# yangzhaojason/DualDiff

Hardware: AMD Instinct MI355X
Metric: denoising-steps/sec, 6-view 224×400 fp16, 50-step DDIM @ 1/2/4/8 MI355X (higher is better)
Workload: dtype fp16; 1 GPU; BASELINE configs[1]: 6-view 224x400 (28x50 latents) multiview UNet + 2 ControlNet branches (ORS panorama + ORS-3D, SFA on), CFG 2.0 -> 12 view-instances/scene, DDIM-50 schedule, random-init weights; scenes_per_gpu=1, parallelism=scene-sharded x1 (no data-path collective), hip_graph=True, streams=3, invariant_conditioning=recomputed every step

## Files before the change

### dualdiff_amd/_native.py

```python
import ctypes
import os

import torch
from ctypes import (POINTER, Structure, c_char_p, c_float, c_int32, c_int64, c_uint32, c_void_p)

from . import _build

DD_F16, DD_BF16, DD_F32 = 0, 1, 2
DD_EPI_NONE, DD_EPI_GEGLU, DD_EPI_SILU = 0, 1, 2


class GemmDesc(Structure):
    _fields_ = [
        ("a", c_void_p), ("a2", c_void_p), ("lda", c_int64), ("lda2", c_int64), ("k1", c_int32),
        ("rows", c_int32), ("n", c_int32), ("k", c_int32),
        ("w", c_void_p), ("bias", c_void_p), ("rowvec", c_void_p),
        ("rows_per_inst", c_int32), ("ld_rowvec", c_int32),
        ("res", c_void_p), ("ldres", c_int64),
        ("out", c_void_p), ("ldc", c_int64),
        ("alpha", c_float), ("accumulate", c_int32), ("epilogue", c_int32),
        ("conv", c_int32), ("hin", c_int32), ("win", c_int32), ("cin", c_int32),
        ("hv", c_int32), ("wv", c_int32), ("hout", c_int32), ("wout", c_int32), ("stride", c_int32),
        ("dtype", c_int32), ("tile", c_int32), ("split_k", c_int32),
        ("ws", c_void_p), ("ws_bytes", c_int64),
        ("ln_colsum", c_void_p), ("ln_bias", c_void_p), ("ln_eps", c_float), ("out_f32", c_int32), ("ln_stats_out", c_void_p), ("ln_stats_in", c_void_p),
        ("out_headmajor_d", c_int32), ("hm_scaled_planes", c_int32), ("hm_scale", c_float),
        ("phase", c_int32),
        ("ln_out", c_void_p), ("ld_ln_out", c_int64), ("lno_gamma", c_void_p), ("lno_beta", c_void_p),
    ]


class AttnDesc(Structure):
    _fields_ = [
        ("q", c_void_p), ("k", c_void_p), ("v", c_void_p), ("o", c_void_p),
        ("ldq", c_int64), ("ldk", c_int64), ("ldv", c_int64), ("ldo", c_int64),
        ("q_batch_stride", c_int64), ("k_batch_stride", c_int64),
        ("v_batch_stride", c_int64), ("o_batch_stride", c_int64),
        ("batch", c_int32), ("heads", c_int32), ("head_dim", c_int32), ("lq", c_int32), ("lk", c_int32),
        ("scale", c_float),
        ("kv_batch_map", c_void_p),
        ("accumulate", c_int32), ("dtype", c_int32), ("variant", c_int32),
        ("q_head_stride", c_int64), ("k_head_stride", c_int64), ("v_head_stride", c_int64),
        ("q_prescaled", c_int32),
# ... 35 lines not shown
        ("w", c_void_p), ("w_scale", c_void_p), ("ldw", c_int64),
        ("bias", c_void_p), ("res", c_void_p), ("ldres", c_int64),
        ("out", c_void_p), ("ldc", c_int64),
        ("rows", c_int32), ("n", c_int32), ("k_padded", c_int32), ("dtype", c_int32),
        ("out_headmajor_d", c_int32), ("hm_scaled_planes", c_int32), ("hm_scale", c_float), ("geglu", c_int32),
    ]


SIGNATURES = {
    "dd_abi_version": (c_int32, []),
    "dd_desc_size": (c_int64, [c_int32]),
    "dd_error_string": (c_char_p, [c_int32]),
    "dd_target_arch": (c_char_p, []),
    "dd_gemm": (c_int32, [POINTER(GemmDesc), c_void_p]),
    "dd_gemm_workspace_bytes": (c_int64, [POINTER(GemmDesc)]),
    "dd_gemm_num_tiles": (c_int32, []),
    "dd_gemm_tile_id": (c_int32, [c_int32]),
    "dd_gemm_kernel_name": (c_char_p, [POINTER(GemmDesc)]),
    "dd_groupnorm_nhwc": (c_int32, [c_void_p, c_int32, c_void_p, c_int32, c_void_p, c_void_p, c_void_p,
                                    c_int32, c_int32, c_int32, c_float, c_int32, c_int32,
                                    c_void_p, c_int64, c_void_p]),
    "dd_groupnorm_workspace_bytes": (c_int64, [c_int32, c_int32]),
    "dd_groupnorm_is_fused": (c_int32, [c_int32, c_int32, c_int32]),
    "dd_layernorm": (c_int32, [c_void_p, c_void_p, c_void_p, c_void_p, c_int64, c_int32, c_float,
                               c_int32, c_void_p]),
    "dd_attention": (c_int32, [POINTER(AttnDesc), c_void_p]),
    "dd_attention_kernel_name": (c_char_p, [POINTER(AttnDesc)]),
    "dd_add": (c_int32, [c_void_p, c_void_p, c_void_p, c_void_p, c_int64, c_int32, c_void_p]),
    "dd_scale": (c_int32, [c_void_p, c_void_p, c_float, c_int64, c_int32, c_void_p]),
    "dd_probe_spin": (c_int32, [c_void_p, c_uint32, c_void_p]),
    "dd_groupnorm_splitk": (c_int32, [c_void_p, c_int32, c_void_p, c_void_p, c_int32, c_void_p, c_int64, c_void_p,
                                      c_void_p, c_void_p, c_void_p, c_int32, c_int32, c_int32, c_int32, c_float, c_int32,
                                      c_int32, c_void_p]),
    "dd_xattn320": (c_int32, [POINTER(XAttnDesc), c_void_p]),
    "dd_nchw_to_nhwc_views": (c_int32, [c_void_p, c_void_p, c_int32, c_int32, c_int32, c_int32, c_int32, c_int32, c_int32,
                                        c_void_p]),
    "dd_fourier_embed_strided": (c_int32, [c_void_p, c_void_p, c_int64, c_int32, POINTER(c_float), c_int32, c_int32,
                                           c_int32, c_int32, c_int32, c_int64, c_int64, c_int64, c_int64, c_void_p]),
# ... 82 lines not shown
```

### dualdiff_amd/csrc/dd_common.h

```cpp
#pragma once
#include <hip/hip_runtime.h>
#include <stdint.h>
#include <atomic>
#include "../../include/dualdiff_hip.h"

typedef float f32x4 __attribute__((ext_vector_type(4)));
typedef _Float16 f16x8 __attribute__((ext_vector_type(8)));
typedef __bf16 bf16x8 __attribute__((ext_vector_type(8)));
typedef _Float16 f16x4 __attribute__((ext_vector_type(4)));
typedef __bf16 bf16x4 __attribute__((ext_vector_type(4)));
typedef short s16x4 __attribute__((ext_vector_type(4)));
typedef uint32_t u32x4 __attribute__((ext_vector_type(4)));
typedef uint32_t u32x2 __attribute__((ext_vector_type(2)));

#define DD_WAVE 64

template <typename T> struct dd_vec;
template <> struct dd_vec<_Float16> { using v8 = f16x8; using v4 = f16x4; };
template <> struct dd_vec<__bf16>   { using v8 = bf16x8; using v4 = bf16x4; };

__device__ __forceinline__ f32x4 dd_mfma16(f16x8 a, f16x8 b, f32x4 c) {
#ifdef DD_DBG_NOMFMA
  asm volatile("" ::"v"(a), "v"(b));
  return c;
// ... 59 lines not shown
__device__ __forceinline__ float dd_geglu_f(float h, float g) {
#ifdef DD_DBG_GEGLU_CHEAP
  return h * g;
#endif
  const float ax = fabsf(g);
  const float t = __builtin_amdgcn_rcpf(fmaf(0.3275911f * 0.70710678118654752440f, ax, 1.0f));
  float p = fmaf(0.5f * 1.061405429f, t, 0.5f * -1.453152027f);
  p = fmaf(p, t, 0.5f * 1.421413741f);
  p = fmaf(p, t, 0.5f * -0.284496736f);
  p = fmaf(p, t, 0.5f * 0.254829592f);
  const float e = __builtin_amdgcn_exp2f((-0.5f * 1.4426950408889634f) * (g * g));
  const float q = (p * t) * e;
  return h * fmaf(-ax, q, fmaxf(g, 0.0f));
}

__device__ __forceinline__ float dd_wave_sum(float v) {
#pragma unroll
  for (int o = 32; o > 0; o >>= 1) v += __shfl_xor(v, o, 64);
  return v;
}
__device__ __forceinline__ float dd_wave_max(float v) {
#pragma unroll
  for (int o = 32; o > 0; o >>= 1) v = fmaxf(v, __shfl_xor(v, o, 64));
  return v;
}

static inline void dd_clear_error() { (void)hipGetLastError(); }
static inline int dd_check_launch() {
  return hipGetLastError() == hipSuccess ? DD_OK : DD_ERR_LAUNCH;
}
// ... 12 lines not shown
```

### dualdiff_amd/csrc/gemm.hip

```cpp
#include "dd_common.h"
#include "dd_debug.h"
#include <type_traits>

namespace {

constexpr int BK = 64;

struct GemmParams {
  const void* a; const void* a2; int64_t lda, lda2; int k1;
  int rows, n, k;
  const void* w; const void* bias; const void* rowvec; int rows_per_inst, ld_rowvec;
  const void* res; int64_t ldres;
  void* out; int64_t ldc;
  float alpha; int accumulate; int act;
  int hin, win, cin, hv, wv, hout, wout, stride, upsample;
  float scale_h, scale_w;
  int k_per_split;
  float* partial;
  int tiles_m, tiles_n;
  uint32_t a_bytes, a2_bytes, w_bytes;
  uint32_t out_bytes, res_bytes;
  int g_per_tile, chunks_per_split;
  int band_rows, bands; float inv_bands;
  const float* ln_colsum; const float* ln_bias; float ln_eps;
  int out_f32;
  float* stat_out;
  const float* stat_in;
  int hm_d, hm_planes; float hm_scale;
  int persist;
  uint64_t* dbg_stamps;
  float inv_hw, inv_wout, inv_rpi;
  void* ln_out; int64_t ld_ln_out;
  const void* lno_gamma; const void* lno_beta;
  float inv_tiles_n, inv_hm_d;
  uint32_t ln_out_bytes;
};

__device__ __forceinline__ int dd_fdiv(int n, float inv) { return (int)(((float)n + 0.5f) * inv); }


template <typename T>
__device__ __forceinline__ void store8(const GemmParams& p, int64_t row, int col, float (&v)[8]) {
  if (p.hm_d) {
    const int plane = col / p.hm_d;
    if (plane < p.hm_planes) {
#pragma unroll
      for (int e = 0; e < 8; ++e) v[e] *= p.hm_scale;
    }
    dd_st16(reinterpret_cast<T*>(p.out) + ((int64_t)plane * p.rows + row) * p.hm_d + (col - plane * p.hm_d),
            dd_pack8<T>(v));
// ... 42 lines not shown
    for (int i = 0; i < 8; ++i) v[i] += b[i];
  }
  store8<T>(p, row, col, v);
}

__device__ __forceinline__ int xcd_remap(int bid, int nwg) {
  const int xcd = bid & 7;
  const int q = nwg >> 3, r = nwg & 7;
  const int base = (xcd < r) ? xcd * (q + 1) : r * (q + 1) + (xcd - r) * q;
  return base + (bid >> 3);
}

template <typename T, int TM, int TN, bool GEGLU>
__device__ __forceinline__ void store_tile(const GemmParams& p, f32x4 (&acc)[TN][TM], int block_m0,
                                           int block_n0, int wave_m, int wave_n, int lane, int row_end,
                                           const float* ln_mean = nullptr, const float* ln_rstd = nullptr) {
  const int q = lane >> 4;
  const int c = lane & 15;
  const int row0 = block_m0 + wave_m * (TM * 16) + c;
  if constexpr (GEGLU) {
    constexpr int TH = TN / 2;
    constexpr int NG = TH / 2;
    const int col0 = block_n0 + wave_n * (TH * 16) + q * (4 * TH);
    u32x4 bh[NG], bg[NG];
    f32x4 lsh[NG][2], lsg[NG][2], lbh[NG][2], lbg[NG][2];
    if (ln_mean) {
#pragma unroll
      for (int g8 = 0; g8 < NG; ++g8) {
        const int col = min(col0 + g8 * 8, p.n - 8);
#pragma unroll
        for (int h2 = 0; h2 < 2; ++h2) {
// ... 58 lines not shown
      for (int tm = 0; tm < TM; ++tm) {
        const int row = row0 + tm * 16;
        if (row >= row_end) continue;
#pragma unroll
        for (int g8 = 0; g8 < NG; ++g8) {
          const int col = col0 + g8 * 8;
          if (col >= p.n) continue;
          float* dst = p.partial + ((int64_t)blockIdx.z * p.rows + row) * p.n + col;
          *reinterpret_cast<f32x4*>(dst) = acc[g8 * 2][tm];
          *reinterpret_cast<f32x4*>(dst + 4) = acc[g8 * 2 + 1][tm];
        }
      }
      return;
    }
    constexpr int TMB = (TM >= 4 && TM % 2 == 0) ? TM / 2 : TM;
    u32x4 rb[NG];
    int colc[NG];
#pragma unroll
    for (int g8 = 0; g8 < NG; ++g8) colc[g8] = min(col0 + g8 * 8, p.n - 8);
    if (p.bias) {
#pragma unroll
      for (int g8 = 0; g8 < NG; ++g8) rb[g8] = dd_ld16(reinterpret_cast<const T*>(p.bias) + colc[g8]);
    }
    f32x4 lcs[NG][2], lcb[NG][2];
    if (ln_mean) {
#pragma unroll
      for (int g8 = 0; g8 < NG; ++g8)
#pragma unroll
        for (int h2 = 0; h2 < 2; ++h2) {
          lcs[g8][h2] = *reinterpret_cast<const f32x4*>(p.ln_colsum + colc[g8] + 4 * h2);
// ... 55 lines not shown
#pragma unroll
          for (int e = 0; e < 8; ++e) v[e] *= p.alpha;
          if (p.res) {
            dd_unpack8<T>(rr[t2][g8], b);
#pragma unroll
            for (int e = 0; e < 8; ++e) v[e] += b[e];
          }
          if (p.act == DD_EPI_SILU) {
#pragma unroll
            for (int e = 0; e < 8; ++e) v[e] = dd_silu_f(v[e]);
          }
          if (p.accumulate) {
            dd_unpack8<T>(ra[t2][g8], b);
#pragma unroll
            for (int e = 0; e < 8; ++e) v[e] += b[e];
          }
          store8<T>(p, row, col, v);
          if (p.stat_out) {
#pragma unroll
            for (int e = 0; e < 8; ++e) { st_s += v[e]; st_q += v[e] * v[e]; }
          }
        }
        }
        if constexpr (TN == 2 || TN == 4) {
          if (p.stat_out) {
            st_s += __shfl_xor(st_s, 16, 64);  st_q += __shfl_xor(st_q, 16, 64);
            if (TN == 2) { st_s += __shfl_xor(st_s, 32, 64);  st_q += __shfl_xor(st_q, 32, 64); }
            const int gcol = block_n0 + wave_n * (TN * 16) + (TN == 2 ? 0 : (q >> 1) * 32);
            const bool writer = TN == 2 ? q == 0 : (q & 1) == 0;
            if (writer && row < row_end && gcol < p.n) {
              float* dst = p.stat_out + ((int64_t)row * (p.n >> 5) + (gcol >> 5)) * 2;
              dst[0] = st_s;
              dst[1] = st_q;
            }
          }
        }
      }
    }
  }
}

template <typename T, int WAVES_M, int WAVES_N, int TM, int TN, bool CONV, bool GEGLU>
__global__ __launch_bounds__(64 * WAVES_M * WAVES_N)
void dd_gemm_kernel(const GemmParams p) {
  using V8 = typename dd_vec<T>::v8;
  constexpr int NT = 64 * WAVES_M * WAVES_N;
  constexpr int BM = WAVES_M * TM * 16;
  constexpr int BN = WAVES_N * TN * 16;
  constexpr int BN_OUT = GEGLU ? BN / 2 : BN;
  constexpr int XI = BM * 8 / NT;
  constexpr int WI = BN * 8 / NT;
// ... 1735 lines not shown
  if constexpr (NW == 8 && GRP == 1) {
    if (late) main_loop(std::true_type{});
    else main_loop(std::false_type{});
  } else {
    main_loop(std::false_type{});
  }
  DD_STAMP(4);
  if (late && nsteps > 0) {
#pragma unroll
    for (int j = 0; j < TM; ++j)
#pragma unroll
      for (int ks = 0; ks < 2; ++ks)
#pragma unroll
        for (int i = 0; i < TN; ++i) acc[i][j] = C3_MFMA(wf[ks][i], xf[ks][j], acc[i][j]);
  }
  store_tile<T, TM, TN, false>(p, acc, row0, block_n0, wave_m, wave_n, lane, min(p.rows, row0 + vrows));
  DD_STAMP_FLUSH(p);
  C3_SEG_FLUSH(p, wave, lane, nsteps);
}

template <typename T>
__global__ __launch_bounds__(256)
void dd_splitk_reduce_kernel(const GemmParams p, int nsplit) {
  const int64_t groups_per_row = p.n / 8;
  const int64_t total = (int64_t)p.rows * groups_per_row;
  for (int64_t g = (int64_t)blockIdx.x * blockDim.x + threadIdx.x; g < total;
       g += (int64_t)gridDim.x * blockDim.x) {
    const int row = (int)(g / groups_per_row);
    const int col = (int)(g - (int64_t)row * groups_per_row) * 8;
    float v[8] = {0, 0, 0, 0, 0, 0, 0, 0};
    for (int z = 0; z < nsplit; ++z) {
// ... 422 lines not shown

}

extern "C" int dd_gemm_num_tiles(void) { return kNumTiles; }
extern "C" int dd_gemm_tile_id(int index) { return (index >= 0 && index < kNumTiles) ? kTiles[index].id : -1; }

constexpr int64_t DD_COUNTER_BYTES = 65536;

extern "C" int64_t dd_gemm_workspace_bytes(const dd_gemm_desc* d) {
  if (validate(d) != DD_OK) return 0;
  const Plan pl = make_plan(d);
  if (pl.unsupported || pl.split <= 1) return 0;
  return DD_COUNTER_BYTES + (int64_t)pl.split * d->rows * d->n * (int64_t)sizeof(float);
}

extern "C" const char* dd_gemm_kernel_name(const dd_gemm_desc* d) {
  if (validate(d) != DD_OK) return "invalid";
  const Plan pl = make_plan(d);
  if (pl.unsupported) return "unsupported";
  const TileCfg& t = kTiles[pl.tile_idx];
  if (t.stages < 0) {
    const bool band = t.stages == -3;
    const int nsw = (t.id == 31 || band) ? 5 : (t.id >= 37 ? 6 : (t.id >= 35 ? 3 : 4));
    snprintf(g_kname, sizeof(g_kname), "dd_conv3s_kernel<%s, %d, %d, %d, %d, %d, %d, %s> split=%d grid=%dx%d tile=%s",
             d->dtype == DD_F16 ? "_Float16" : "__bf16", t.wm, t.wn, t.tm, t.tn, nsw, (t.id >= 37 && !band) ? 3 : 1,
             band ? "true" : "false", pl.split, pl.tiles_m, pl.tiles_n, t.name);
    return g_kname;
  }
  if (t.stages >= 100) {
    snprintf(g_kname, sizeof(g_kname), "dd_gemm%d_kernel<%s, %d, %d, %d, %d, %d, %s> split=%d grid=%dx%d tile=%s",
// ... 54 lines not shown
      p.a2_bytes = d->a2 ? (uint32_t)((((int64_t)d->rows - 1) * d->lda2 + (d->k - d->k1)) * 2) : 0u;
    }
  }
  {
    const int64_t ob = (((int64_t)d->rows - 1) * d->ldc + d->n) * 2, rb = (((int64_t)d->rows - 1) * d->ldres + d->n) * 2;
    const bool fits = ob < ((int64_t)1 << 31) && (!d->res || rb < ((int64_t)1 << 31));
    p.out_bytes = fits ? (uint32_t)ob : 0u;
    p.res_bytes = fits && d->res ? (uint32_t)rb : 0u;
  }
  p.persist = 0;
  p.inv_tiles_n = 1.0f / (float)(pl.tiles_n > 0 ? pl.tiles_n : 1);
  p.inv_hm_d = d->out_headmajor_d > 0 ? 1.0f / (float)d->out_headmajor_d : 1.0f;
  p.ln_out_bytes = d->ln_out ? (uint32_t)((((int64_t)d->rows - 1) * d->ld_ln_out + d->n) * 2) : 0u;
  p.partial = nullptr;
  p.dbg_stamps = nullptr;
  DD_STAMP_HOST(p, d);
  if (pl.split > 1) {
    const int64_t need = DD_COUNTER_BYTES + (int64_t)pl.split * d->rows * d->n * (int64_t)sizeof(float);
    if (!d->ws || d->ws_bytes < need) return DD_ERR_WORKSPACE;
    p.partial = reinterpret_cast<float*>(reinterpret_cast<char*>(d->ws) + DD_COUNTER_BYTES);
  }
  hipStream_t s = reinterpret_cast<hipStream_t>(stream);
  dd_clear_error();
  if (d->dtype == DD_F16) return launch_dtype<_Float16>(d, p, pl, s);
  return launch_dtype<__bf16>(d, p, pl, s);
}
```

### dualdiff_amd/csrc/norm.hip

```cpp
#include "dd_common.h"
#include <atomic>

namespace {

constexpr int GN_THREADS = 256;
constexpr int GN_MAX_SPLIT = 64;
constexpr int GN_MAX_C = 4096;

struct GnParams {
  const void* x1; const void* x2; int c1, c2, c;
  const void* gamma; const void* beta; void* y;
  int m, hw, groups, cpg; float eps; int silu;
  float* ws;
  int nsplit, pix_per_split;
  const float* sk_part; int sk_nsplit; int64_t sk_rows;
  const void* sk_bias; const void* sk_rowvec; int sk_ld_rowvec;
  const void* sk_res; int64_t sk_ldres;
  void* sk_xout;
};

struct GnMap { int cv_count, pl_count, cv, pl; bool active; };
__device__ __forceinline__ GnMap gn_map(int c) {
  GnMap mp;
  mp.cv_count = c >> 3;
  if (mp.cv_count >= GN_THREADS) {
    mp.pl_count = 1; mp.cv = threadIdx.x; mp.pl = 0; mp.active = true;
  } else {
    mp.pl_count = GN_THREADS / mp.cv_count;
    mp.cv = threadIdx.x % mp.cv_count;
    mp.pl = threadIdx.x / mp.cv_count;
    mp.active = mp.pl < mp.pl_count;
  }
  return mp;
}
// ... 105 lines not shown
          const int t = mp.cv_count >= GN_THREADS ? (c - cv0) : pl * mp.cv_count + c;
          if (s_g0[t] == g) { gsum += s_a0[t]; gsq += s_b0[t]; }
          if (s_g1[t] == g) { gsum += s_a1[t]; gsq += s_b1[t]; }
        }
      }
    }
    __syncthreads();
  }
  if (threadIdx.x < p.groups) {
    float* dst = p.ws + (((int64_t)inst * p.nsplit + split) * p.groups + threadIdx.x) * 2;
    dst[0] = gsum;
    dst[1] = gsq;
  }
}

template <typename T>
__global__ __launch_bounds__(GN_THREADS)
void dd_gn_apply_kernel(const GnParams p) {
  __shared__ float s_mean[64], s_rstd[64];
  __shared__ float s_ps[GN_THREADS], s_pq[GN_THREADS];
  const int split = blockIdx.x, inst = blockIdx.y;
  const GnMap mp = gn_map(p.c);
  const int p0 = split * p.pix_per_split;
  const int p1 = min(p.hw, p0 + p.pix_per_split);
  const float my_pivot = (int)threadIdx.x < p.groups ? gn_pivot<T>(p, inst, threadIdx.x) : 0.f;
  const int cv_first = mp.cv;
  const int ch_first = min(cv_first, mp.cv_count - 1) << 3;
  u32x4 pre[GN_UNROLL];
  const bool pre_ok = mp.active && cv_first < mp.cv_count && p0 + mp.pl + (GN_UNROLL - 1) * mp.pl_count < p1;
  if (pre_ok) {
#pragma unroll
    for (int u = 0; u < GN_UNROLL; ++u)
      pre[u] = dd_ld16(gn_src<T>(p, (int64_t)inst * p.hw + p0 + mp.pl + u * mp.pl_count, ch_first));
  }
  {
    const int g = threadIdx.x % p.groups;
    const int chunk = threadIdx.x / p.groups;
    const int nchunk = GN_THREADS / p.groups;
    float s = 0.f, ss = 0.f;
    if (chunk < nchunk) {
      const float* src = p.ws + ((int64_t)inst * p.nsplit * p.groups + g) * 2;
      for (int i = chunk; i < p.nsplit; i += nchunk) {
        s += src[(int64_t)i * p.groups * 2];
        ss += src[(int64_t)i * p.groups * 2 + 1];
      }
    }
    s_ps[threadIdx.x] = s;
    s_pq[threadIdx.x] = ss;
    __syncthreads();
    if (threadIdx.x < p.groups) {
// ... 349 lines not shown
  int cpb, vpp, plc, nv, kred, threads;
  if (gn_fused_plan(hw, c, groups, &cpb, &vpp, &plc, &nv, &kred, &threads)) {
    dim3 fgrid(c / cpb, m);
    if (threads == 256) {
      if (dtype == DD_F16) hipLaunchKernelGGL((dd_gn_fused_kernel<_Float16, 256, GNF_NV_SMALL>), fgrid, dim3(256), 0, s, p, cpb, vpp, plc, nv, kred);
      else hipLaunchKernelGGL((dd_gn_fused_kernel<__bf16, 256, GNF_NV_SMALL>), fgrid, dim3(256), 0, s, p, cpb, vpp, plc, nv, kred);
    } else {
      if (dtype == DD_F16) hipLaunchKernelGGL((dd_gn_fused_kernel<_Float16, 1024, GNF_NV_BIG>), fgrid, dim3(1024), 0, s, p, cpb, vpp, plc, nv, kred);
      else hipLaunchKernelGGL((dd_gn_fused_kernel<__bf16, 1024, GNF_NV_BIG>), fgrid, dim3(1024), 0, s, p, cpb, vpp, plc, nv, kred);
    }
    return dd_check_launch();
  }
  dim3 grid(p.nsplit, m);
  if (dtype == DD_F16) {
    hipLaunchKernelGGL(dd_gn_stats_kernel<_Float16>, grid, dim3(GN_THREADS), 0, s, p);
    hipLaunchKernelGGL(dd_gn_apply_kernel<_Float16>, grid, dim3(GN_THREADS), 0, s, p);
  } else {
    hipLaunchKernelGGL(dd_gn_stats_kernel<__bf16>, grid, dim3(GN_THREADS), 0, s, p);
    hipLaunchKernelGGL(dd_gn_apply_kernel<__bf16>, grid, dim3(GN_THREADS), 0, s, p);
  }
  return dd_check_launch();
}

extern "C" int dd_groupnorm_splitk(const float* partial, int32_t nsplit, const void* bias, const void* rowvec,
                                   int32_t ld_rowvec, const void* res, int64_t ldres, void* x_out,
                                   const void* gamma, const void* beta, void* y, int32_t m, int32_t hw, int32_t c,
                                   int32_t groups, float eps, int32_t apply_silu, int32_t dtype, dd_stream_t stream) {
  if (!partial || !gamma || !beta || !y || nsplit < 2 || nsplit > 64) return DD_ERR_BAD_ARG;
  if (m <= 0 || hw <= 0 || groups <= 0 || groups > 64 || c <= 0 || (c & 7) || c % groups || c > GN_MAX_C) return DD_ERR_BAD_ARG;
  if (c / groups < 4) return DD_ERR_UNSUPPORTED;
  if (dtype != DD_F16 && dtype != DD_BF16) return DD_ERR_BAD_ARG;
  if (!dd_aligned16(partial) || !dd_aligned16(y) || !dd_aligned16(gamma) || !dd_aligned16(beta) ||
      (bias && !dd_aligned16(bias)) || (rowvec && (!dd_aligned16(rowvec) || (ld_rowvec & 7))) ||
      (res && (!dd_aligned16(res) || (ldres & 7))) || (x_out && !dd_aligned16(x_out))) return DD_ERR_BAD_ARG;
  int cpb, vpp, plc, nv, kred, threads;
// ... 51 lines not shown
```

### dualdiff_amd/networks/layers.py

```python
import math

import torch
import torch.nn as nn

from .. import ops as O


CACHE_EPOCH = [0]


class _Cached(nn.Module):

    def _drop_cache(self):
        CACHE_EPOCH[0] += 1
        for k in [k for k in self.__dict__ if k.startswith("_pk_")]:
            del self.__dict__[k]

    def _apply(self, fn, *a, **k):
        self._drop_cache()
        return super()._apply(fn, *a, **k)

    def _load_from_state_dict(self, *a, **k):
        self._drop_cache()
        return super()._load_from_state_dict(*a, **k)
# ... 148 lines not shown
    @property
    def cin_pad(self):
        return (self.in_channels + 7) // 8 * 8

    @property
    def packed(self):
        if "_pk_w" not in self.__dict__:
            w = self.weight.detach().permute(0, 2, 3, 1)
            if self.cin_pad != self.in_channels:
                wp = w.new_zeros((self.out_channels, 3, 3, self.cin_pad))
                wp[..., :self.in_channels] = w
                w = wp
            self.__dict__["_pk_w"] = w.reshape(self.out_channels, 9 * self.cin_pad).contiguous()
        return self.__dict__["_pk_w"]

    def run(self, x2d, m, h, w, up_size=None, **kw):
        return O.conv3x3(x2d, self.packed, self.bias, m, h, w, stride=self.stride, up_size=up_size, **kw)

    def out_hw(self, h, w, up_size=None):
        hv, wv = (h, w) if up_size is None else up_size
        return (hv - 1) // self.stride + 1, (wv - 1) // self.stride + 1

    def forward(self, x):
        x2d, m, h, w = to_nhwc(x)
        if x2d.shape[1] != self.cin_pad:
            x2d = torch.nn.functional.pad(x2d, (0, self.cin_pad - x2d.shape[1]))
        ho, wo = self.out_hw(h, w)
        return as_nchw_view(self.run(x2d, m, h, w), m, ho, wo)


class GroupNorm(nn.Module):
    def __init__(self, num_groups, num_channels, eps=1e-5):
        super().__init__()
        self.num_groups, self.num_channels, self.eps = num_groups, num_channels, eps
        self.weight = nn.Parameter(torch.empty(num_channels))
        self.bias = nn.Parameter(torch.empty(num_channels))

    def run(self, x2d, m, hw, silu, x2=None):
        hit = getattr(x2d, "_gn_cache", None)
        if hit is not None:
            del x2d._gn_cache
            if hit[0] is self and hit[1] == bool(silu) and x2 is None:
                return hit[2]
        if getattr(x2d, "_unwritten", False):
            raise RuntimeError("this conv output was folded into its GroupNorm and never written")
        return O.groupnorm(x2d, self.weight, self.bias, m, hw, self.num_groups, self.eps, silu, x2=x2)


class LayerNorm(nn.Module):
    def __init__(self, dim, eps=1e-5):
        super().__init__()
        self.eps = eps
        self.weight = nn.Parameter(torch.empty(dim))
        self.bias = nn.Parameter(torch.empty(dim))

    def run(self, x2d):
        hit = getattr(x2d, "_ln_cache", None)
        if hit is not None:
            del x2d._ln_cache
            if hit[0] is self:
                return hit[1]
# ... 91 lines not shown
class ResnetBlock2D(nn.Module):

    def __init__(self, in_channels, out_channels, temb_channels, groups=32, eps=1e-5):
        super().__init__()
        self.in_channels, self.out_channels = in_channels, out_channels
        self.norm1 = GroupNorm(groups, in_channels, eps)
        self.conv1 = Conv3x3(in_channels, out_channels)
        self.time_emb_proj = Linear(temb_channels, out_channels)
        self.norm2 = GroupNorm(groups, out_channels, eps)
        self.conv2 = Conv3x3(out_channels, out_channels)
        self.conv_shortcut = Linear(in_channels, out_channels, conv=True) if in_channels != out_channels else None

    def run(self, x, m, h, w, temb_vec, x2=None, extra_res=None, gn_next=None):
        hw = h * w
        a = self.norm1.run(x, m, hw, True, x2=x2)
        hid = self.conv1.run(a, m, h, w, rowvec=temb_vec, gn_next=(self.norm2, True, False))
        a = self.norm2.run(hid, m, hw, True)
        if self.conv_shortcut is not None:
            sc = self.conv_shortcut.run(x, a2=x2, res=extra_res)
        elif extra_res is not None:
            sc = O.add(x, extra_res)
        else:
            sc = x
        return self.conv2.run(a, m, h, w, res=sc, gn_next=None if gn_next is None else (gn_next, False, True))


class Downsample2D(nn.Module):
    def __init__(self, channels):
        super().__init__()
        self.conv = Conv3x3(channels, channels, stride=2)


class Upsample2D(nn.Module):
    def __init__(self, channels):
        super().__init__()
        self.conv = Conv3x3(channels, channels)


class HIPAttnProcessor:
# ... 480 lines not shown
```

### dualdiff_amd/ops.py

```python
import collections as _collections
import ctypes
import threading as _threading

import torch

from . import _native
from ._native import DD_BF16, DD_EPI_GEGLU, DD_EPI_NONE, DD_EPI_SILU, DD_F16, AttnDesc, Gemm8Desc, GemmDesc, XAttnDesc

_WS = {}
_WS_MIN_BYTES = 64 << 20


class KernelTimer:

    def __init__(self, shapes=False):
        self.records = []
        self.shapes = shapes
        self.overhead_ms = 0.0
        self.empty_bracket_ms = 0.0
        self.probe_ms = 0.0

    def calibrate(self, n=48, probe_us=15.0):
        lib = _native.load()
        st = torch.cuda.current_stream()
# ... 264 lines not shown


class workspace_owner:

    def __init__(self, token):
        self.token = token

    def __enter__(self):
        self.prev = getattr(_WS_OWNER, "token", None)
        _WS_OWNER.token = self.token

    def __exit__(self, *exc):
        _WS_OWNER.token = self.prev


def workspace(nbytes, device, kind="gemm"):
    owner = getattr(_WS_OWNER, "token", None)
    key = (device.type, device.index if device.index is not None else torch.cuda.current_device(),
           torch.cuda.current_stream().cuda_stream if owner is None else ("owner", owner), kind)
    ws = _WS.get(key)
    need = max(int(nbytes), _WS_MIN_BYTES)
    capturing = torch.cuda.is_current_stream_capturing()
    if ws is None or ws.numel() * 4 < need:
        if capturing:
            raise RuntimeError("workspace would have to grow during graph capture; run one eager "
                               "warm-up step first")
        if ws is not None and key in _WS_IN_GRAPH:
            _WS_RETIRED.append(ws)
            _WS_IN_GRAPH.discard(key)
        ws = torch.zeros((need + 3) // 4, dtype=torch.float32, device=device)
        _WS[key] = ws
    if capturing:
        _WS_IN_GRAPH.add(key)
    return ws


# ... 30 lines not shown
        _TIMER.stop(e0, name + suffix, flops, nbytes, staged)
        return
    slab = 4.0 * split * rows * n
    d.phase = 1
    e0 = _TIMER.start()
    _native.check(lib.dd_gemm(ctypes.byref(d), _stream()), what)
    _TIMER.stop(e0, name + suffix, flops, nbytes + slab, staged)
    d.phase = 2
    e0 = _TIMER.start()
    _native.check(lib.dd_gemm(ctypes.byref(d), _stream()), what)
    _TIMER.stop(e0, "dd_splitk_reduce_kernel", 0.0, slab + 2.0 * rows * n)
    d.phase = 0


def _forget_derived(t):
    for a in ("_ln_cache", "_ln_out", "_ln_stats", "_gn_cache", "_unwritten"):
        if hasattr(t, a):
            delattr(t, a)


def _rows2d(t):
    if t.dim() != 2 or t.stride(1) != 1:
        raise ValueError("expected a 2-D tensor with unit inner stride, got shape %s stride %s"
                         % (tuple(t.shape), t.stride()))
    return t


def gemm(a, w, bias=None, *, a2=None, res=None, rowvec=None, rows_per_inst=1, alpha=1.0,
         out=None, accumulate=False, epilogue=DD_EPI_NONE, tile=0, split_k=0, ln=None, out_f32=False,
         ln_stats=False, head_major=None, ln_out=None):
    lib = _native.load()
# ... 94 lines not shown
    else:
        _native.check(lib.dd_gemm(ctypes.byref(d), _stream()), "gemm")
    if stats_out is not None:
        out._ln_stats = stats_out
    if ln_second is not None:
        out._ln_out = ln_second
    return hm_out if hm_out is not None else out


_THIN_CONV = _os.environ.get("DD_THIN_CONV", "1") != "0"
GN_SPLITK = _os.environ.get("DD_GN_SPLITK", "0") == "1"


LN_OUT_TILE = int(_os.environ.get("DD_LN_OUT_TILE", "0"))


def thin_conv_ok(cin, cout, stride, m):
    return _THIN_CONV and (cin, cout, stride) in ((8, 16, 1), (16, 16, 1), (16, 32, 2), (32, 32, 1), (8, 32, 1), (16, 32, 1),
                                                  (16, 16, 2), (8, 16, 2), (32, 16, 1)) and m <= 65535


def conv3x3(x, w, bias, m, hin, win, *, stride=1, up_size=None, rowvec=None, res=None,
            alpha=1.0, out=None, accumulate=False, epilogue=DD_EPI_NONE, tile=0, split_k=0, gn_next=None):
    lib = _native.load()
    _need_gpu(x, w, bias, res, rowvec, out)
    x = _rows2d(x)
    cin = x.shape[1]
    if not x.is_contiguous() or x.shape[0] != m * hin * win:
        raise ValueError("conv input must be contiguous (m*h*w, cin)")
    hv, wv = (hin, win) if up_size is None else (int(up_size[0]), int(up_size[1]))
    hout = (hv + 2 - 3) // stride + 1
    wout = (wv + 2 - 3) // stride + 1
    cout = w.shape[0]
    if w.shape[1] != 9 * cin or not w.is_contiguous():
        raise ValueError("conv weight must be contiguous [cout, 9*cin]")
    rows = m * hout * wout
    if out is None:
        out = torch.empty((rows, cout), dtype=x.dtype, device=x.device)
# ... 23 lines not shown
        d.res = res.data_ptr(); d.ldres = res.stride(0)
    out = _rows2d(out)
    d.out = out.data_ptr(); d.ldc = out.stride(0)
    d.alpha = alpha; d.accumulate = int(accumulate); d.epilogue = epilogue
    d.conv = 1
    d.hin, d.win, d.cin, d.hv, d.wv = hin, win, cin, hv, wv
    d.hout, d.wout, d.stride = hout, wout, stride
    d.dtype = _dt(x); d.tile = tile; d.split_k = split_k
    if tile == 0 and split_k == 0:
        d.tile, d.split_k, _ = _autotune(lib, d, ("c", m, hin, win, cin, cout, stride, hv, wv, d.dtype),
                                      (rows, cout), x.dtype, x.device, warm=(x, res))
    need = lib.dd_gemm_workspace_bytes(ctypes.byref(d))
    if need > 0 or _DBG_STAMP_WS:
        ws = workspace(need, x.device)
        d.ws = ws.data_ptr(); d.ws_bytes = ws.numel() * 4
    if gn_next is not None and GN_SPLITK and need > 0 and alpha == 1.0 and not accumulate and epilogue == DD_EPI_NONE:
        gmod, gsilu, want_x = gn_next
        _, split = _kname(lib, d)
        if split > 1 and lib.dd_groupnorm_is_fused(hout * wout, cout, gmod.num_groups):
            y = torch.empty((rows, cout), dtype=x.dtype, device=x.device)
            d.phase = 1
            e0 = _TIMER.start() if _TIMER is not None else None
            _native.check(lib.dd_gemm(ctypes.byref(d), _stream()), "conv3x3")
            if e0 is not None:
                name = _kname(lib, d)[0]
                _TIMER.stop(e0, name + (" conv %dx%dx%d" % (rows, cout, 9 * cin) if _TIMER.shapes else ""),
                            2.0 * rows * cout * 9 * cin, 2.0 * (x.numel() + w.numel()) + 4.0 * split * rows * cout,
                            _staged_bytes(lib, d))
                e0 = _TIMER.start()
            rc = lib.dd_groupnorm_splitk(ctypes.c_void_p(ws.data_ptr() + 65536), split, _ptr(bias), _ptr(rowvec),
# ... 1 lines not shown
                                         res.stride(0) if res is not None else 0, _ptr(out) if want_x else None,
                                         _ptr(gmod.weight), _ptr(gmod.bias), _ptr(y), m, hout * wout, cout,
                                         gmod.num_groups, float(gmod.eps), int(gsilu), _dt(x), _stream())
            _native.check(rc, "groupnorm_splitk")
            if e0 is not None:
                _TIMER.stop(e0, "dd_gn_splitk_kernel", 0.0, 4.0 * split * rows * cout + 2.0 * rows * cout * (2 if want_x else 1))
            out._gn_cache = (gmod, bool(gsilu), y)
            if not want_x:
                out._unwritten = True
            return out
    if _TIMER is not None:
        _timed_gemm(lib, d, "conv3x3", " conv %dx%dx%d" % (rows, cout, 9 * cin) if _TIMER.shapes else "",
                    2.0 * rows * cout * 9 * cin,
                    2.0 * (x.numel() + w.numel() + rows * cout * (1 + (1 if d.res else 0) + (1 if d.accumulate else 0))),
                    rows, cout)
        return out
    _native.check(lib.dd_gemm(ctypes.byref(d), _stream()), "conv3x3")
    return out


def groupnorm(x, gamma, beta, m, hw, groups, eps, silu, x2=None, out=None):
    lib = _native.load()
    _need_gpu(x, gamma, beta, x2, out)
    c1 = x.shape[1]
    c2 = x2.shape[1] if x2 is not None else 0
    if not x.is_contiguous() or (x2 is not None and not x2.is_contiguous()):
        raise ValueError("groupnorm inputs must be contiguous")
    if out is None:
        out = torch.empty((m * hw, c1 + c2), dtype=x.dtype, device=x.device)
    need = lib.dd_groupnorm_workspace_bytes(m, groups)
    ws = workspace(need, x.device, "gn")
    e0 = _TIMER.start() if _TIMER is not None else None
    rc = lib.dd_groupnorm_nhwc(_ptr(x), c1, _ptr(x2), c2, _ptr(gamma), _ptr(beta), _ptr(out),
                               m, hw, groups, eps, int(silu), _dt(x), _ptr(ws), ws.numel() * 4,
                               _stream())
    _native.check(rc, "groupnorm")
    if e0 is not None:
        th = lib.dd_groupnorm_is_fused(hw, c1 + c2, groups)
        _TIMER.stop(e0, "dd_gn_fused_kernel<%s, %d, 8>" % ("f16" if x.dtype == torch.float16 else "bf16", th) if th
                    else "dd_gn_stats_kernel + dd_gn_apply_kernel (2 launches)",
                    0.0, (4.0 if th else 6.0) * out.numel())
    return out


# ... 573 lines not shown
```

### include/dualdiff_hip.h

```cpp
#ifndef DUALDIFF_HIP_H
#define DUALDIFF_HIP_H

#include <stdint.h>

#ifdef __cplusplus
extern "C" {
#endif

#define DD_ABI_VERSION 4

enum { DD_F16 = 0, DD_BF16 = 1 };

enum {
  DD_OK = 0,
  DD_ERR_BAD_ARG = -1,
  DD_ERR_UNSUPPORTED = -2,
  DD_ERR_LAUNCH = -3,
  DD_ERR_WORKSPACE = -4
};

typedef void* dd_stream_t;

int dd_abi_version(void);
int64_t dd_desc_size(int which);
// ... 30 lines not shown
  int64_t ws_bytes;
  const void* ln_colsum;
  const void* ln_bias;
  float ln_eps;
  int32_t out_f32;
  void* ln_stats_out;
  const void* ln_stats_in;
  int32_t out_headmajor_d;
  int32_t hm_scaled_planes;
  float hm_scale;
  int32_t phase;
  void* ln_out;
  int64_t ld_ln_out;
  const void* lno_gamma;
  const void* lno_beta;
} dd_gemm_desc;

int dd_gemm(const dd_gemm_desc* d, dd_stream_t stream);
int64_t dd_gemm_workspace_bytes(const dd_gemm_desc* d);
int dd_gemm_num_tiles(void);
int dd_gemm_tile_id(int index);
const char* dd_gemm_kernel_name(const dd_gemm_desc* d);

int dd_groupnorm_nhwc(const void* x1, int32_t c1, const void* x2, int32_t c2,
                      const void* gamma, const void* beta, void* y,
                      int32_t m, int32_t hw, int32_t groups, float eps,
                      int32_t apply_silu, int32_t dtype, void* ws, int64_t ws_bytes,
                      dd_stream_t stream);
int64_t dd_groupnorm_workspace_bytes(int32_t m, int32_t groups);
int dd_groupnorm_is_fused(int32_t hw, int32_t c, int32_t groups);
int dd_groupnorm_splitk(const float* partial, int32_t nsplit, const void* bias, const void* rowvec, int32_t ld_rowvec,
                        const void* res, int64_t ldres, void* x_out, const void* gamma, const void* beta, void* y,
                        int32_t m, int32_t hw, int32_t c, int32_t groups, float eps, int32_t apply_silu, int32_t dtype,
                        dd_stream_t stream);

int dd_layernorm(const void* x, const void* gamma, const void* beta, void* y,
                 int64_t rows, int32_t c, float eps, int32_t dtype, dd_stream_t stream);

typedef struct dd_attn_desc {
  const void* q; const void* k; const void* v; void* o;
  int64_t ldq, ldk, ldv, ldo;
  int64_t q_batch_stride, k_batch_stride, v_batch_stride, o_batch_stride;
  int32_t batch, heads, head_dim, lq, lk;
  float scale;
  const int32_t* kv_batch_map;
// ... 129 lines not shown
```

Baseline: 91.65 steps/s.

## Emit per-channel GroupNorm partial statistics from conv3x3 epilogue and skip the stats pass

The banded conv3x3 GEMM epilogue now computes per-column Welford mean/M2 partials per tile-row segment, reducing them across lanes and waves through LDS, and writes them to a side buffer. A new groupnorm entry point merges these partials per channel, then per group, inside the apply kernel, so the separate stats kernel and its full re-read of the conv output are skipped. This adds epilogue ALU work, two block barriers and extra LDS use in the GEMM, and requires the plan to match one specific tile configuration. It falls back to the old path when unsupported.

```diff
diff --git a/dualdiff_amd/_native.py b/dualdiff_amd/_native.py
--- a/dualdiff_amd/_native.py
+++ b/dualdiff_amd/_native.py
@@ -27,6 +27,7 @@
         ("out_headmajor_d", c_int32), ("hm_scaled_planes", c_int32), ("hm_scale", c_float),
         ("phase", c_int32),
         ("ln_out", c_void_p), ("ld_ln_out", c_int64), ("lno_gamma", c_void_p), ("lno_beta", c_void_p),
+        ("gn_part", c_void_p), ("gn_part_bytes", c_int64),
     ]
 
 
@@ -92,6 +93,7 @@
     "dd_target_arch": (c_char_p, []),
     "dd_gemm": (c_int32, [POINTER(GemmDesc), c_void_p]),
     "dd_gemm_workspace_bytes": (c_int64, [POINTER(GemmDesc)]),
+    "dd_gemm_gn_part_bytes": (c_int64, [POINTER(GemmDesc), POINTER(c_int32)]),
     "dd_gemm_num_tiles": (c_int32, []),
     "dd_gemm_tile_id": (c_int32, [c_int32]),
     "dd_gemm_kernel_name": (c_char_p, [POINTER(GemmDesc)]),
@@ -100,6 +102,9 @@
                                     c_void_p, c_int64, c_void_p]),
     "dd_groupnorm_workspace_bytes": (c_int64, [c_int32, c_int32]),
     "dd_groupnorm_is_fused": (c_int32, [c_int32, c_int32, c_int32]),
+    "dd_groupnorm_partials": (c_int32, [c_void_p, c_int32, c_void_p, c_int32, c_void_p, c_int32, c_void_p, c_int32,
+                                        c_void_p, c_void_p, c_void_p, c_int32, c_int32, c_int32, c_float, c_int32,
+                                        c_int32, c_void_p]),
     "dd_layernorm": (c_int32, [c_void_p, c_void_p, c_void_p, c_void_p, c_int64, c_int32, c_float,
                                c_int32, c_void_p]),
     "dd_attention": (c_int32, [POINTER(AttnDesc), c_void_p]),
diff --git a/dualdiff_amd/csrc/dd_common.h b/dualdiff_amd/csrc/dd_common.h
--- a/dualdiff_amd/csrc/dd_common.h
+++ b/dualdiff_amd/csrc/dd_common.h
@@ -97,6 +97,16 @@
   return h * fmaf(-ax, q, fmaxf(g, 0.0f));
 }
 
+__device__ __forceinline__ float dd_chan_frac(float na, float nb) {
+  const float n = na + nb;
+  return n > 0.f ? nb / n : 0.f;
+}
+__device__ __forceinline__ void dd_chan_add(float& mean, float& m2, float na, float fb, float mb, float qb) {
+  const float d = mb - mean;
+  mean += d * fb;
+  m2 += qb + d * d * na * fb;
+}
+
 __device__ __forceinline__ float dd_wave_sum(float v) {
 #pragma unroll
   for (int o = 32; o > 0; o >>= 1) v += __shfl_xor(v, o, 64);
diff --git a/dualdiff_amd/csrc/gemm.hip b/dualdiff_amd/csrc/gemm.hip
--- a/dualdiff_amd/csrc/gemm.hip
+++ b/dualdiff_amd/csrc/gemm.hip
@@ -34,6 +34,7 @@
   const void* lno_gamma; const void* lno_beta;
   float inv_tiles_n, inv_hm_d;
   uint32_t ln_out_bytes;
+  float* gn_part;
 };
 
 __device__ __forceinline__ int dd_fdiv(int n, float inv) { return (int)(((float)n + 0.5f) * inv); }
@@ -106,7 +107,8 @@
 template <typename T, int TM, int TN, bool GEGLU>
 __device__ __forceinline__ void store_tile(const GemmParams& p, f32x4 (&acc)[TN][TM], int block_m0,
                                            int block_n0, int wave_m, int wave_n, int lane, int row_end,
-                                           const float* ln_mean = nullptr, const float* ln_rstd = nullptr) {
+                                           const float* ln_mean = nullptr, const float* ln_rstd = nullptr,
+                                           int gn_seg = -1, int gn_waves_m = 0, float* gn_lds = nullptr) {
   const int q = lane >> 4;
   const int c = lane & 15;
   const int row0 = block_m0 + wave_m * (TM * 16) + c;
@@ -195,6 +197,10 @@
       return;
     }
     constexpr int TMB = (TM >= 4 && TM % 2 == 0) ? TM / 2 : TM;
+    const bool gn = NG == 1 && gn_seg >= 0 && p.gn_part;
+    float gm[8], gq[8];
+#pragma unroll
+    for (int e = 0; e < 8; ++e) { gm[e] = 0.f; gq[e] = 0.f; }
     u32x4 rb[NG];
     int colc[NG];
 #pragma unroll
@@ -280,6 +286,17 @@
             dd_unpack8<T>(ra[t2][g8], b);
 #pragma unroll
             for (int e = 0; e < 8; ++e) v[e] += b[e];
+          }
+          if (gn) {
+            float f[8];
+            dd_unpack8<T>(dd_pack8<T>(v), f);
+            const float inv = 1.0f / (float)(tm + 1);
+#pragma unroll
+            for (int e = 0; e < 8; ++e) {
+              const float d = f[e] - gm[e];
+              gm[e] += d * inv;
+              gq[e] += d * (f[e] - gm[e]);
+            }
           }
           store8<T>(p, row, col, v);
           if (p.stat_out) {
@@ -301,6 +318,45 @@
             }
           }
         }
+      }
+    }
+    if (gn) {
+      float na = 0.f;
+#pragma unroll
+      for (int tm = 0; tm < TM; ++tm) na += row0 + tm * 16 < row_end ? 1.f : 0.f;
+#pragma unroll
+      for (int o = 1; o < 16; o <<= 1) {
+        const float nb = __shfl_xor(na, o, 64);
+        const float fb = dd_chan_frac(na, nb);
+#pragma unroll
+        for (int e = 0; e < 8; ++e)
+          dd_chan_add(gm[e], gq[e], na, fb, __shfl_xor(gm[e], o, 64), __shfl_xor(gq[e], o, 64));
+        na += nb;
+      }
+      __syncthreads();
+      float* mine = gn_lds + ((wave_n * 4 + q) * gn_waves_m + wave_m) * 17;
+      if (c == 0) {
+        mine[0] = na;
+#pragma unroll
+        for (int e = 0; e < 8; ++e) { mine[1 + e] = gm[e]; mine[9 + e] = gq[e]; }
+      }
+      __syncthreads();
+      if (wave_m == 0 && c == 0 && col0 < p.n) {
+        for (int w = 1; w < gn_waves_m; ++w) {
+          const float* o = mine + w * 17;
+          const float nb = o[0];
+          const float fb = dd_chan_frac(na, nb);
+#pragma unroll
+          for (int e = 0; e < 8; ++e) dd_chan_add(gm[e], gq[e], na, fb, o[1 + e], o[9 + e]);
+          na += nb;
+        }
+        float* rec = p.gn_part + (int64_t)gn_seg * 3 * p.n + col0;
+        *reinterpret_cast<f32x4*>(rec) = f32x4{na, na, na, na};
+        *reinterpret_cast<f32x4*>(rec + 4) = f32x4{na, na, na, na};
+        *reinterpret_cast<f32x4*>(rec + p.n) = f32x4{gm[0], gm[1], gm[2], gm[3]};
+        *reinterpret_cast<f32x4*>(rec + p.n + 4) = f32x4{gm[4], gm[5], gm[6], gm[7]};
+        *reinterpret_cast<f32x4*>(rec + 2 * p.n) = f32x4{gq[0], gq[1], gq[2], gq[3]};
+        *reinterpret_cast<f32x4*>(rec + 2 * p.n + 4) = f32x4{gq[4], gq[5], gq[6], gq[7]};
       }
     }
   }
@@ -2066,7 +2122,8 @@
 #pragma unroll
         for (int i = 0; i < TN; ++i) acc[i][j] = C3_MFMA(wf[ks][i], xf[ks][j], acc[i][j]);
   }
-  store_tile<T, TM, TN, false>(p, acc, row0, block_n0, wave_m, wave_n, lane, min(p.rows, row0 + vrows));
+  store_tile<T, TM, TN, false>(p, acc, row0, block_n0, wave_m, wave_n, lane, min(p.rows, row0 + vrows), nullptr, nullptr,
+                               BAND && p.gn_part ? tile_m : -1, WAVES_M, reinterpret_cast<float*>(smem));
   DD_STAMP_FLUSH(p);
   C3_SEG_FLUSH(p, wave, lane, nsteps);
 }
@@ -2519,6 +2576,18 @@
   return DD_COUNTER_BYTES + (int64_t)pl.split * d->rows * d->n * (int64_t)sizeof(float);
 }
 
+int64_t gn_part_bytes(const dd_gemm_desc* d, const Plan& pl, int32_t* segs_per_inst) {
+  if (pl.unsupported || pl.split != 1 || kTiles[pl.tile_idx].stages != -3 || kTiles[pl.tile_idx].tn != 2) return 0;
+  if (d->accumulate || d->out_f32 || d->out_headmajor_d || d->ln_stats_out || d->epilogue == DD_EPI_GEGLU) return 0;
+  if (segs_per_inst) *segs_per_inst = pl.bands;
+  return (int64_t)pl.tiles_m * 3 * d->n * (int64_t)sizeof(float);
+}
+
+extern "C" int64_t dd_gemm_gn_part_bytes(const dd_gemm_desc* d, int32_t* segs_per_inst) {
+  if (validate(d) != DD_OK) return 0;
+  return gn_part_bytes(d, make_plan(d), segs_per_inst);
+}
+
 extern "C" const char* dd_gemm_kernel_name(const dd_gemm_desc* d) {
   if (validate(d) != DD_OK) return "invalid";
   const Plan pl = make_plan(d);
@@ -2603,6 +2672,13 @@
   p.ln_out_bytes = d->ln_out ? (uint32_t)((((int64_t)d->rows - 1) * d->ld_ln_out + d->n) * 2) : 0u;
   p.partial = nullptr;
   p.dbg_stamps = nullptr;
+  p.gn_part = nullptr;
+  if (d->gn_part) {
+    const int64_t gb = gn_part_bytes(d, pl, nullptr);
+    if (gb == 0) return DD_ERR_UNSUPPORTED;
+    if (d->gn_part_bytes < gb || !dd_aligned16(d->gn_part)) return DD_ERR_BAD_ARG;
+    p.gn_part = reinterpret_cast<float*>(d->gn_part);
+  }
   DD_STAMP_HOST(p, d);
   if (pl.split > 1) {
     const int64_t need = DD_COUNTER_BYTES + (int64_t)pl.split * d->rows * d->n * (int64_t)sizeof(float);
diff --git a/dualdiff_amd/csrc/norm.hip b/dualdiff_amd/csrc/norm.hip
--- a/dualdiff_amd/csrc/norm.hip
+++ b/dualdiff_amd/csrc/norm.hip
@@ -17,7 +17,10 @@
   const void* sk_bias; const void* sk_rowvec; int sk_ld_rowvec;
   const void* sk_res; int64_t sk_ldres;
   void* sk_xout;
+  const float* pt1; const float* pt2; int segs1, segs2;
 };
+
+constexpr int GN_PART_MAX_C = 1280;
 
 struct GnMap { int cv_count, pl_count, cv, pl; bool active; };
 __device__ __forceinline__ GnMap gn_map(int c) {
@@ -153,16 +156,17 @@
   }
 }
 
-template <typename T>
+template <typename T, bool PART>
 __global__ __launch_bounds__(GN_THREADS)
 void dd_gn_apply_kernel(const GnParams p) {
   __shared__ float s_mean[64], s_rstd[64];
-  __shared__ float s_ps[GN_THREADS], s_pq[GN_THREADS];
+  __shared__ float s_ps[PART ? 3 * GN_PART_MAX_C : 2 * GN_THREADS];
+  float* s_pq = s_ps + GN_THREADS;
   const int split = blockIdx.x, inst = blockIdx.y;
   const GnMap mp = gn_map(p.c);
   const int p0 = split * p.pix_per_split;
   const int p1 = min(p.hw, p0 + p.pix_per_split);
-  const float my_pivot = (int)threadIdx.x < p.groups ? gn_pivot<T>(p, inst, threadIdx.x) : 0.f;
+  const float my_pivot = !PART && (int)threadIdx.x < p.groups ? gn_pivot<T>(p, inst, threadIdx.x) : 0.f;
   const int cv_first = mp.cv;
   const int ch_first = min(cv_first, mp.cv_count - 1) << 3;
   u32x4 pre[GN_UNROLL];
@@ -172,7 +176,34 @@
     for (int u = 0; u < GN_UNROLL; ++u)
       pre[u] = dd_ld16(gn_src<T>(p, (int64_t)inst * p.hw + p0 + mp.pl + u * mp.pl_count, ch_first));
   }
-  {
+  if constexpr (PART) {
+    float* s_n = s_ps;
+    float* s_m = s_ps + GN_PART_MAX_C;
+    float* s_q = s_ps + 2 * GN_PART_MAX_C;
+    for (int ch = threadIdx.x; ch < p.c; ch += GN_THREADS) {
+      const bool two = ch >= p.c1;
+      const int cc = two ? p.c2 : p.c1, segs = two ? p.segs2 : p.segs1;
+      const float* rec = (two ? p.pt2 + (ch - p.c1) : p.pt1 + ch) + (int64_t)inst * segs * 3 * cc;
+      float n = 0.f, mean = 0.f, m2 = 0.f;
+      for (int sg = 0; sg < segs; ++sg, rec += 3 * cc) {
+        const float nb = rec[0];
+        dd_chan_add(mean, m2, n, dd_chan_frac(n, nb), rec[cc], rec[2 * cc]);
+        n += nb;
+      }
+      s_n[ch] = n; s_m[ch] = mean; s_q[ch] = m2;
+    }
+    __syncthreads();
+    if (threadIdx.x < p.groups) {
+      float n = 0.f, mean = 0.f, m2 = 0.f;
+      for (int ch = threadIdx.x * p.cpg; ch < (threadIdx.x + 1) * p.cpg; ++ch) {
+        const float nb = s_n[ch];
+        dd_chan_add(mean, m2, n, dd_chan_frac(n, nb), s_m[ch], s_q[ch]);
+        n += nb;
+      }
+      s_mean[threadIdx.x] = mean;
+      s_rstd[threadIdx.x] = rsqrtf(fmaxf(m2 / n, 0.f) + p.eps);
+    }
+  } else {
     const int g = threadIdx.x % p.groups;
     const int chunk = threadIdx.x / p.groups;
     const int nchunk = GN_THREADS / p.groups;
@@ -552,11 +583,39 @@
   dim3 grid(p.nsplit, m);
   if (dtype == DD_F16) {
     hipLaunchKernelGGL(dd_gn_stats_kernel<_Float16>, grid, dim3(GN_THREADS), 0, s, p);
-    hipLaunchKernelGGL(dd_gn_apply_kernel<_Float16>, grid, dim3(GN_THREADS), 0, s, p);
+    hipLaunchKernelGGL((dd_gn_apply_kernel<_Float16, false>), grid, dim3(GN_THREADS), 0, s, p);
   } else {
     hipLaunchKernelGGL(dd_gn_stats_kernel<__bf16>, grid, dim3(GN_THREADS), 0, s, p);
-    hipLaunchKernelGGL(dd_gn_apply_kernel<__bf16>, grid, dim3(GN_THREADS), 0, s, p);
-  }
+    hipLaunchKernelGGL((dd_gn_apply_kernel<__bf16, false>), grid, dim3(GN_THREADS), 0, s, p);
+  }
+  return dd_check_launch();
+}
+
+extern "C" int dd_groupnorm_partials(const void* x1, int32_t c1, const float* part1, int32_t segs1,
+                                     const void* x2, int32_t c2, const float* part2, int32_t segs2,
+                                     const void* gamma, const void* beta, void* y, int32_t m, int32_t hw, int32_t groups,
+                                     float eps, int32_t apply_silu, int32_t dtype, dd_stream_t stream) {
+  if (!x1 || !part1 || !gamma || !beta || !y || segs1 <= 0) return DD_ERR_BAD_ARG;
+  if (c2 < 0 || (c2 > 0 && (!x2 || !part2 || segs2 <= 0))) return DD_ERR_BAD_ARG;
+  const int c = c1 + c2;
+  if (m <= 0 || hw <= 0 || groups <= 0 || groups > 64 || c1 <= 0) return DD_ERR_BAD_ARG;
+  if ((c1 & 7) || (c2 & 7) || c % groups != 0) return DD_ERR_BAD_ARG;
+  if (c > GN_PART_MAX_C) return DD_ERR_UNSUPPORTED;
+  if (c / groups < 4) return DD_ERR_UNSUPPORTED;
+  if (dtype != DD_F16 && dtype != DD_BF16) return DD_ERR_BAD_ARG;
+  if (!dd_aligned16(x1) || (x2 && !dd_aligned16(x2)) || !dd_aligned16(y) ||
+      !dd_aligned16(gamma) || !dd_aligned16(beta)) return DD_ERR_BAD_ARG;
+  GnParams p{};
+  p.x1 = x1; p.x2 = x2; p.c1 = c1; p.c2 = c2; p.c = c;
+  p.gamma = gamma; p.beta = beta; p.y = y;
+  p.m = m; p.hw = hw; p.groups = groups; p.cpg = c / groups; p.eps = eps; p.silu = apply_silu;
+  p.pt1 = part1; p.pt2 = part2; p.segs1 = segs1; p.segs2 = c2 > 0 ? segs2 : 0;
+  p.nsplit = gn_plan(hw, c, &p.pix_per_split);
+  hipStream_t s = reinterpret_cast<hipStream_t>(stream);
+  dd_clear_error();
+  dim3 grid(p.nsplit, m);
+  if (dtype == DD_F16) hipLaunchKernelGGL((dd_gn_apply_kernel<_Float16, true>), grid, dim3(GN_THREADS), 0, s, p);
+  else hipLaunchKernelGGL((dd_gn_apply_kernel<__bf16, true>), grid, dim3(GN_THREADS), 0, s, p);
   return dd_check_launch();
 }
 
diff --git a/dualdiff_amd/networks/layers.py b/dualdiff_amd/networks/layers.py
--- a/dualdiff_amd/networks/layers.py
+++ b/dualdiff_amd/networks/layers.py
@@ -186,8 +186,9 @@
             self.__dict__["_pk_w"] = w.reshape(self.out_channels, 9 * self.cin_pad).contiguous()
         return self.__dict__["_pk_w"]
 
-    def run(self, x2d, m, h, w, up_size=None, **kw):
-        return O.conv3x3(x2d, self.packed, self.bias, m, h, w, stride=self.stride, up_size=up_size, **kw)
+    def run(self, x2d, m, h, w, up_size=None, gn_part=False, **kw):
+        return O.conv3x3(x2d, self.packed, self.bias, m, h, w, stride=self.stride, up_size=up_size,
+                         gn_part=self if gn_part else None, **kw)
 
     def out_hw(self, h, w, up_size=None):
         hv, wv = (h, w) if up_size is None else up_size
@@ -216,7 +217,10 @@
                 return hit[2]
         if getattr(x2d, "_unwritten", False):
             raise RuntimeError("this conv output was folded into its GroupNorm and never written")
-        return O.groupnorm(x2d, self.weight, self.bias, m, hw, self.num_groups, self.eps, silu, x2=x2)
+        parts = [t.__dict__.pop("_gn_part", None) if t is not None else None for t in (x2d, x2)]
+        if parts[0] is None or (x2 is not None and parts[1] is None) or parts[0][2:] != (m, hw):
+            parts = None
+        return O.groupnorm(x2d, self.weight, self.bias, m, hw, self.num_groups, self.eps, silu, x2=x2, parts=parts)
 
 
 class LayerNorm(nn.Module):
@@ -338,7 +342,7 @@
     def run(self, x, m, h, w, temb_vec, x2=None, extra_res=None, gn_next=None):
         hw = h * w
         a = self.norm1.run(x, m, hw, True, x2=x2)
-        hid = self.conv1.run(a, m, h, w, rowvec=temb_vec, gn_next=(self.norm2, True, False))
+        hid = self.conv1.run(a, m, h, w, rowvec=temb_vec, gn_next=(self.norm2, True, False), gn_part=True)
         a = self.norm2.run(hid, m, hw, True)
         if self.conv_shortcut is not None:
             sc = self.conv_shortcut.run(x, a2=x2, res=extra_res)
@@ -346,7 +350,8 @@
             sc = O.add(x, extra_res)
         else:
             sc = x
-        return self.conv2.run(a, m, h, w, res=sc, gn_next=None if gn_next is None else (gn_next, False, True))
+        return self.conv2.run(a, m, h, w, res=sc, gn_next=None if gn_next is None else (gn_next, False, True),
+                              gn_part=gn_next is not None)
 
 
 class Downsample2D(nn.Module):
diff --git a/dualdiff_amd/ops.py b/dualdiff_amd/ops.py
--- a/dualdiff_amd/ops.py
+++ b/dualdiff_amd/ops.py
@@ -302,12 +302,12 @@
         _WS_OWNER.token = self.prev
 
 
-def workspace(nbytes, device, kind="gemm"):
+def workspace(nbytes, device, kind="gemm", floor=_WS_MIN_BYTES):
     owner = getattr(_WS_OWNER, "token", None)
     key = (device.type, device.index if device.index is not None else torch.cuda.current_device(),
            torch.cuda.current_stream().cuda_stream if owner is None else ("owner", owner), kind)
     ws = _WS.get(key)
-    need = max(int(nbytes), _WS_MIN_BYTES)
+    need = max(int(nbytes), floor)
     capturing = torch.cuda.is_current_stream_capturing()
     if ws is None or ws.numel() * 4 < need:
         if capturing:
@@ -368,7 +368,7 @@
 
 
 def _forget_derived(t):
-    for a in ("_ln_cache", "_ln_out", "_ln_stats", "_gn_cache", "_unwritten"):
+    for a in ("_ln_cache", "_ln_out", "_ln_stats", "_gn_cache", "_gn_part", "_unwritten"):
         if hasattr(t, a):
             delattr(t, a)
 
@@ -493,6 +493,8 @@
 
 LN_OUT_TILE = int(_os.environ.get("DD_LN_OUT_TILE", "0"))
 
+GN_PART = _os.environ.get("DD_GN_PART", "1") != "0"
+
 
 def thin_conv_ok(cin, cout, stride, m):
     return _THIN_CONV and (cin, cout, stride) in ((8, 16, 1), (16, 16, 1), (16, 32, 2), (32, 32, 1), (8, 32, 1), (16, 32, 1),
@@ -500,7 +502,7 @@
 
 
 def conv3x3(x, w, bias, m, hin, win, *, stride=1, up_size=None, rowvec=None, res=None,
-            alpha=1.0, out=None, accumulate=False, epilogue=DD_EPI_NONE, tile=0, split_k=0, gn_next=None):
+            alpha=1.0, out=None, accumulate=False, epilogue=DD_EPI_NONE, tile=0, split_k=0, gn_next=None, gn_part=None):
     lib = _native.load()
     _need_gpu(x, w, bias, res, rowvec, out)
     x = _rows2d(x)
@@ -554,6 +556,14 @@
     if need > 0 or _DBG_STAMP_WS:
         ws = workspace(need, x.device)
         d.ws = ws.data_ptr(); d.ws_bytes = ws.numel() * 4
+    part = None
+    if gn_part is not None and GN_PART and need == 0:
+        segs = ctypes.c_int32(0)
+        pbytes = lib.dd_gemm_gn_part_bytes(ctypes.byref(d), ctypes.byref(segs))
+        if pbytes > 0:
+            buf = workspace(pbytes, x.device, ("gn_part", gn_part), floor=0)
+            d.gn_part, d.gn_part_bytes = buf.data_ptr(), buf.numel() * 4
+            part = (buf, segs.value, m, hout * wout)
     if gn_next is not None and GN_SPLITK and need > 0 and alpha == 1.0 and not accumulate and epilogue == DD_EPI_NONE:
         gmod, gsilu, want_x = gn_next
         _, split = _kname(lib, d)
@@ -585,12 +595,14 @@
                     2.0 * rows * cout * 9 * cin,
                     2.0 * (x.numel() + w.numel() + rows * cout * (1 + (1 if d.res else 0) + (1 if d.accumulate else 0))),
                     rows, cout)
-        return out
-    _native.check(lib.dd_gemm(ctypes.byref(d), _stream()), "conv3x3")
-    return out
-
-
-def groupnorm(x, gamma, beta, m, hw, groups, eps, silu, x2=None, out=None):
+    else:
+        _native.check(lib.dd_gemm(ctypes.byref(d), _stream()), "conv3x3")
+    if part is not None:
+        out._gn_part = part
+    return out
+
+
+def groupnorm(x, gamma, beta, m, hw, groups, eps, silu, x2=None, out=None, parts=None):
     lib = _native.load()
     _need_gpu(x, gamma, beta, x2, out)
     c1 = x.shape[1]
@@ -599,6 +611,19 @@
         raise ValueError("groupnorm inputs must be contiguous")
     if out is None:
         out = torch.empty((m * hw, c1 + c2), dtype=x.dtype, device=x.device)
+    if parts is not None:
+        p1, p2 = parts
+        if p1[2:] != (m, hw) or (x2 is not None) != (p2 is not None) or (p2 is not None and p2[2:] != (m, hw)):
+            raise ValueError("GroupNorm partial records do not describe this input")
+        e0 = _TIMER.start() if _TIMER is not None else None
+        rc = lib.dd_groupnorm_partials(_ptr(x), c1, _ptr(p1[0]), p1[1], _ptr(x2), c2, _ptr(p2[0]) if p2 else None,
+                                       p2[1] if p2 else 0, _ptr(gamma), _ptr(beta), _ptr(out), m, hw, groups, eps,
+                                       int(silu), _dt(x), _stream())
+        if rc != -2:
+            _native.check(rc, "groupnorm_partials")
+            if e0 is not None:
+                _TIMER.stop(e0, "dd_gn_apply_kernel (partials)", 0.0, 4.0 * out.numel())
+            return out
     need = lib.dd_groupnorm_workspace_bytes(m, groups)
     ws = workspace(need, x.device, "gn")
     e0 = _TIMER.start() if _TIMER is not None else None
diff --git a/include/dualdiff_hip.h b/include/dualdiff_hip.h
--- a/include/dualdiff_hip.h
+++ b/include/dualdiff_hip.h
@@ -68,10 +68,13 @@
   int64_t ld_ln_out;
   const void* lno_gamma;
   const void* lno_beta;
+  void* gn_part;
+  int64_t gn_part_bytes;
 } dd_gemm_desc;
 
 int dd_gemm(const dd_gemm_desc* d, dd_stream_t stream);
 int64_t dd_gemm_workspace_bytes(const dd_gemm_desc* d);
+int64_t dd_gemm_gn_part_bytes(const dd_gemm_desc* d, int32_t* segs_per_inst);
 int dd_gemm_num_tiles(void);
 int dd_gemm_tile_id(int index);
 const char* dd_gemm_kernel_name(const dd_gemm_desc* d);
@@ -83,6 +86,10 @@
                       dd_stream_t stream);
 int64_t dd_groupnorm_workspace_bytes(int32_t m, int32_t groups);
 int dd_groupnorm_is_fused(int32_t hw, int32_t c, int32_t groups);
+int dd_groupnorm_partials(const void* x1, int32_t c1, const float* part1, int32_t segs1,
+                          const void* x2, int32_t c2, const float* part2, int32_t segs2,
+                          const void* gamma, const void* beta, void* y, int32_t m, int32_t hw, int32_t groups,
+                          float eps, int32_t apply_silu, int32_t dtype, dd_stream_t stream);
 int dd_groupnorm_splitk(const float* partial, int32_t nsplit, const void* bias, const void* rowvec, int32_t ld_rowvec,
                         const void* res, int64_t ldres, void* x_out, const void* gamma, const void* beta, void* y,
                         int32_t m, int32_t hw, int32_t c, int32_t groups, float eps, int32_t apply_silu, int32_t dtype,
```

Result: no change. 91.96 steps/s, median of 6 (+0.3%).
